# AdamCodd/local-hyperDB

Measured on AMD Instinct MI355X. Metric: queries/sec, N=10M d=384 fp16 top-100 (single-query stream; p50 latency alongside), higher is better.
Workload: dtype f16; 1 GPU; N=10000000 d=384 fp16 Q=1 cosine_similarity top-100, row-sharded x1; rows_per_gpu=10000000, accumulate=f32, exchange=none

## Files before the change

local-hyperdb_amd/csrc/hdb_api.hip:

```cpp
#include "hdb_common.h"
#include "hdb_quant.h"
#include "hdb_ws.h"
#include "hdb_plan.h"
#include "../../include/hyperdb_hip.h"
#include <string>
#include <cmath>
#include <cstring>
#include <cstdio>
#include <algorithm>
#include <vector>
#include <chrono>
#include <atomic>

static thread_local std::string g_err;
static int fail(int code, const std::string& msg) { g_err = msg; return code; }
#define HIP_TRY(expr)                                                                              \
    do {                                                                                           \
        hipError_t e_ = (expr);                                                                    \
        if (e_ != hipSuccess)                                                                      \
            return fail(HDB_ERR_HIP, std::string(#expr) + ": " + hipGetErrorString(e_));           \
    } while (0)
#define LAUNCH_TRY(expr)                                                                           \
    do {                                                                                           \
        int e_ = (expr);                                                                           \
// ... 31 lines not shown
    uint32_t fused_epoch = 0;
    char* bctl = nullptr;
    char* rec = nullptr;
    size_t rec_bytes = 0;
    int qmode = HDB_QUANT_NONE;
    int8_t* qcodes = nullptr;
    float* qaux = nullptr;
    int64_t q_rows = 0;
    int32_t qP = 0;
    int* qstat = nullptr;
    uint8_t* pnib = nullptr;
    uint32_t* pbit = nullptr;
    float* prec = nullptr;
    int32_t pU = 0;
    bool plane_declined = false;
    bool qauto = false;
    bool qauto_declined = false;
    char* ws = nullptr;
    size_t ws_bytes = 0;
    hdb_options opt;
    int flags_host = -1;
    TopkStats st;
    int64_t st_host_direct = 0;
    const uint32_t* qb_cnt = nullptr;
    int qb_cnt_n = 0;
    int64_t ht_pre_ns = 0, ht_launch_ns = 0, ht_wait_ns = 0, ht_calls = 0;
    std::chrono::steady_clock::time_point ht_l0, ht_l1;
    int64_t ht_attr_ns = 0;
    int64_t profile = 0;
    std::vector<hipEvent_t> ev_pool;
    size_t ev_used = 0;
};

static int ensure_ws(hdb_index* ix, size_t bytes) {
    if (bytes <= ix->ws_bytes) return HDB_OK;
    if (ix->ws) { HIP_TRY(hipDeviceSynchronize()); HIP_TRY(hipFree(ix->ws)); ix->ws = nullptr; ix->ws_bytes = 0; }
    bytes = align_up(bytes + (bytes >> 2), 1 << 20);
    HIP_TRY(hipMalloc((void**)&ix->ws, bytes));
    ix->ws_bytes = bytes;
    return HDB_OK;
}
template <typename WS, typename... Ext>
static int ws_lay(hdb_index* ix, WS& w, Ext... ext) {
    const int rc = ensure_ws(ix, ws_bytes_for<WS>(ext...));
    if (rc) return rc;
    Bump b(ix->ws, ix->ws_bytes);
    w.lay(b, ext...);
    if (b.off > b.cap) return fail(HDB_ERR_NOMEM, "workspace: a layout ran past the size it reported");
    return HDB_OK;
}

extern "C" int hdb_version(void) { return 107; }
extern "C" const char* hdb_last_error(void) { return g_err.c_str(); }

static int build_caches(hdb_index* ix, hipStream_t st) {
    if (ix->n > ix->cache_rows) {
        if (ix->inv_norm) { HIP_TRY(hipDeviceSynchronize()); HIP_TRY(hipFree(ix->inv_norm)); HIP_TRY(hipFree(ix->sqnorm)); }
        const int64_t rows = ix->n + ix->n / 4 + 64;
        HIP_TRY(hipMalloc((void**)&ix->inv_norm, rows * sizeof(float)));
        HIP_TRY(hipMalloc((void**)&ix->sqnorm, rows * sizeof(float)));
        ix->cache_rows = rows;
    }
    HIP_TRY(hipMemsetAsync(ix->nan_flag, 0, sizeof(int), st));
    if (ix->n > 0) LAUNCH_TRY(hdb_launch_rownorm(ix->V, ix->n, ix->d, ix->dtype, ix->inv_norm, ix->sqnorm, ix->nan_flag, st));
    ix->flags_host = -1;
    ix->bits_valid = false; ix->bits_done = 0;
    ix->pscale_valid = false; ix->pscale_done = 0;
    ix->build_stream = st;
    return HDB_OK;
}

static double quant_gamma(int d) {
    const double u = std::ldexp(1.0, -24), m = (double)(d + 8) * u;
    return m / (1.0 - m) * (1.0 + std::ldexp(1.0, -20));
}
// ... 344 lines not shown
    else if (!strcmp(name, "host_poll")) ix->opt.host_poll = value;
    else if (!strcmp(name, "dyn_tiles")) ix->opt.dyn_tiles = value;
    else if (!strcmp(name, "dyn_min_mb")) ix->opt.dyn_min_mb = std::max<int64_t>(0, value);
    else if (!strcmp(name, "dyn_heavy")) ix->opt.dyn_heavy = value;
    else if (!strcmp(name, "fused_timeout_us")) ix->opt.fused_timeout_us = std::max<int64_t>(1, value);
    else if (!strcmp(name, "bits_fused")) ix->opt.bits_fused = value;
    else if (!strcmp(name, "bits_local")) ix->opt.bits_local = value;
    else if (!strcmp(name, "fused_max_q")) ix->opt.fused_max_q = value;
    else if (!strcmp(name, "f32_min_q")) ix->opt.f32_min_q = value;
    else if (!strcmp(name, "f32_split")) ix->opt.f32_split = value;
    else if (!strcmp(name, "f32_split_min_q")) ix->opt.f32_split_min_q = value;
    else if (!strcmp(name, "bf16_ks_min_q")) ix->opt.bf16_ks_min_q = value;
    else if (!strcmp(name, "f8_ks_min_q")) ix->opt.f8_ks_min_q = value < 0 ? -1 : value;
    else if (!strcmp(name, "f8_lds_min_q")) ix->opt.f8_lds_min_q = value < 0 ? -1 : value;
    else if (!strcmp(name, "bf16_quant")) ix->opt.bf16_quant = value ? 1 : 0;
    else if (!strcmp(name, "f8_lds_waves")) { if (value == 0 || value == 4 || value == 8) ix->opt.f8_lds_waves = value; }
    else if (!strcmp(name, "bits_max_q")) ix->opt.bits_max_q = value;
    else if (!strcmp(name, "use_quant")) ix->opt.use_quant = value;
    else if (!strcmp(name, "quant_min_n")) ix->opt.quant_min_n = value;
    else if (!strcmp(name, "auto_quant")) ix->opt.auto_quant = value;
    else if (!strcmp(name, "quant_batch_min_n")) ix->opt.quant_batch_min_n = value;
    else if (!strcmp(name, "quant_batch_kernel")) ix->opt.quant_batch_kernel = value ? 1 : 0;
    else if (!strcmp(name, "quant_max_k")) ix->opt.quant_max_k = std::max<int64_t>(1, std::min<int64_t>(value, 128));
    else if (!strcmp(name, "use_plane")) ix->opt.use_plane = value;
    else if (!strcmp(name, "plane_min_n")) ix->opt.plane_min_n = value;
    else if (!strcmp(name, "plane_cap_rows")) ix->opt.plane_cap_rows = std::max<int64_t>(0, value);
    else if (!strcmp(name, "plane_wg_per_cu")) ix->opt.plane_wg_per_cu = std::max<int64_t>(0, std::min<int64_t>(value, 8));
    else if (!strcmp(name, "use_subset")) ix->opt.use_subset = value;
    else if (!strcmp(name, "subset_min_n")) ix->opt.subset_min_n = value < 0 ? -1 : value;
    else if (!strcmp(name, "subset_ratio")) ix->opt.subset_ratio = value < 0 ? -1 : std::max<int64_t>(1, value);
    else if (!strcmp(name, "profile")) { ix->profile = value; ix->ev_used = 0; }
    else if (!strcmp(name, "host_timing_reset")) { ix->ht_pre_ns = ix->ht_launch_ns = ix->ht_wait_ns = ix->ht_calls = ix->ht_attr_ns = 0; }
    else return fail(HDB_ERR_ARG, std::string("hdb_set_option: unknown option ") + name);
    return HDB_OK;
}

extern "C" int hdb_get_stat(hdb_index* ix, const char* name, int64_t* value) {
    if (!ix || !name || !value) return fail(HDB_ERR_ARG, "hdb_get_stat: null argument");
    if (!strcmp(name, "sample_rows")) *value = ix->st.sample_rows;
    else if (!strcmp(name, "sample_m")) *value = ix->st.sample_m;
    else if (!strcmp(name, "path")) *value = ix->st.path;
    else if (!strcmp(name, "chunks")) *value = ix->st.chunks;
    else if (!strcmp(name, "mfma")) *value = ix->st.mfma;
    else if (!strcmp(name, "f32_split")) *value = ix->st.f32s;
    else if (!strcmp(name, "f8_lds")) *value = ix->st.f8_lds;
    else if (!strcmp(name, "f8_lds_min_q")) *value = f8_lds_first_q(ix->opt, ix->dtype, ix->d);
    else if (!strcmp(name, "host_direct")) *value = ix->st_host_direct;
    else if (!strcmp(name, "fused")) *value = ix->st.fused;
    else if (!strcmp(name, "local")) *value = ix->st.local;
    else if (!strcmp(name, "cand_cap")) *value = HDB_CAND_CAP;
    else if (!strcmp(name, "quant")) *value = ix->st.quant;
    else if (!strcmp(name, "quant_auto")) *value = (ix->qmode == HDB_QUANT_I8 && ix->qauto) ? 1 : 0;
    else if (!strcmp(name, "quant_bytes")) *value = ix->qmode == HDB_QUANT_I8 ? ix->n * (int64_t)(ix->qP + 12) : 0;
    else if (!strcmp(name, "plane")) *value = ix->st.plane;
    else if (!strcmp(name, "plane_blocks")) *value = ix->st.plane_blocks;
    else if (!strcmp(name, "subset")) *value = ix->st.subset;
    else if (!strcmp(name, "subset_rows")) *value = ix->subset_m;
    else if (!strcmp(name, "plane_bytes")) *value = (ix->qmode == HDB_QUANT_I8 && ix->pnib) ? ix->n * (int64_t)plane_row_bytes(ix->qP) : 0;
    else if (!strcmp(name, "plane_survivors") || !strcmp(name, "plane_overflows")) {
        int h[HDB_QSTAT_WORDS] = {0, 0, 0, 0};
        if (ix->qstat) {
            HIP_TRY(hipSetDevice(ix->device));
            HIP_TRY(hipDeviceSynchronize());
            HIP_TRY(hipMemcpy(h, ix->qstat, sizeof(h), hipMemcpyDeviceToHost));
        }
        *value = name[6] == 's' ? (ix->st.plane ? (int64_t)(uint32_t)h[1] : 0) : (int64_t)(uint32_t)h[2];
    }
    else if (!strcmp(name, "quant_cands")) {
        int h = 0;
        if (ix->st.quant && ix->qstat) {
            HIP_TRY(hipSetDevice(ix->device));
            HIP_TRY(hipDeviceSynchronize());
            HIP_TRY(hipMemcpy(&h, ix->qstat, sizeof(int), hipMemcpyDeviceToHost));
        }
        *value = h;
    }
// ... 194 lines not shown
    }
    if (p.plane_wanted && !ix->pnib) {
        const int rc = plane_rows(ix, 0, ix->n, st);
        if (rc) return rc;
        *declined = ix->pnib == nullptr;
    }
    return HDB_OK;
}

static int quant_topk(hdb_index* ix, const TopkArgs& c, const TopkPlan& p) {
    const void* dev_Q = c.Q; const int32_t nq = c.nq, k = c.k; const int metric = c.metric; hipStream_t st = c.st;
    int64_t* dev_idx = c.idx; float* dev_score = c.score; int32_t* dev_status = c.status;
    const uint32_t kk = p.kk; const bool mflavour = p.mflavour, use_pl = p.plane_wanted;
    const int64_t n = ix->n;
    const uint32_t m = 16;
    const QuantSample sp = p.qs;
    QuantWs w;
    int rc = quant_ws_lay(ix, w, nq, quant_hi_cap(ix, nq), mflavour);
    if (rc) return rc;
    uint32_t* qstat = reinterpret_cast<uint32_t*>(ix->qstat);
    uint32_t* pl_cnt = use_pl ? qstat + 1 : nullptr;
    const size_t crow = (size_t)nq * HDB_CAND_CAP;
    const int nsub = p.nsub;
    rc = quant_query_prep(ix, (const float*)dev_Q, nq, w, mflavour, ix->qstat, nsub ? w.cnt : nullptr, pl_cnt, st);
    if (rc) return rc;
    QuantArgs a; quant_base_args(ix, a, w.qcodes, w.qaux, w.qinv, metric, nq);
    a.ntiles = sp.s_tiles; a.tile_stride = sp.s_stride; a.scores = w.sbuf; a.ld = sp.ld_s;
    a.wmax = w.wmax; a.nsub = nsub; a.thr_out = w.thr;
    a.pl_hi = use_pl ? reinterpret_cast<float*>(w.pl_list) : nullptr;
    if (use_pl && (!a.pl_hi || sp.s_rows > (int64_t)quant_hi_cap(ix, nq))) return fail(HDB_ERR_ARG, "quant_topk: no list for the sampled rows");
    LAUNCH_TRY(hdb_launch_quant_scan(&a, 0, (int)ix->opt.max_blocks, st));
    if (!nsub) LAUNCH_TRY(hdb_launch_sample_thr(w.sbuf, sp.s_rows, sp.ld_s, nq, m, w.thr, w.cnt, nullptr, st));
    a.ntiles = (n + 15) / 16; a.tile_stride = 1; a.scores = nullptr; a.ld = 0;
    a.thr = w.thr; a.cnt = w.cnt; a.cand = w.cand; a.cap = HDB_CAND_CAP;
    const bool has_bias = ix->bias != nullptr || ix->mask != nullptr;
    if (mflavour) {
        a.V = (const char*)ix->V; a.row_bytes = ix->d * 2; a.G = w.G;
        a.ginv = metric == HDB_COSINE ? w.ginv : nullptr; a.gbias = has_bias ? w.gbias : nullptr;
    }
    prof_begin(ix, st);
    if (use_pl) {
        a.pl_nib = ix->pnib; a.pl_bit = ix->pbit; a.pl_rec = ix->prec; a.pl_units = ix->pU;
        a.pl_cnt = pl_cnt; a.pl_cap = p.pl_cap;
        a.pl_s_tiles = (uint32_t)sp.s_tiles; a.pl_s_stride = (uint32_t)sp.s_stride;
        LAUNCH_TRY(hdb_launch_quant_plane_scan(&a, 0, p.pl_blocks, st));
    } else {
        LAUNCH_TRY(hdb_launch_quant_scan(&a, 1, (int)ix->opt.max_blocks, st));
    }
    prof_end(ix, st);
    if (mflavour) {
        ScanArgs s; memset(&s, 0, sizeof(s));
        s.V = w.G; s.n = (int64_t)crow; s.d = ix->d; s.Q = dev_Q; s.metric = metric; s.inv_norm = w.ginv; s.qinv = w.qinv;
        s.bias = has_bias ? w.gbias : nullptr; s.mask = nullptr; s.nq = nq;
        s.tile_stride = 1; s.ntiles = (int64_t)crow / hdb_mfma_tile_rows(ix->dtype, ix->d); s.cap = HDB_CAND_CAP;
        s.scores = w.gsc; s.ld = (int64_t)crow;
        LAUNCH_TRY(hdb_launch_mfma_scan(&s, ix->dtype, 0, nq, w.q16, w.ginv, w.qsq, w.qscl, (int)ix->opt.max_blocks, (int)ix->opt.mfma_variant, st, nullptr));
    } else {
        LAUNCH_TRY(hdb_launch_quant_rescore(ix->V, ix->d, ix->dtype, (const float*)dev_Q, nq, metric, ix->inv_norm, w.qinv, ix->bias, ix->mask,
                                            w.cand, w.cnt, HDB_CAND_CAP, st));
    }
    LAUNCH_TRY(hdb_launch_quant_finalize(w.cand, w.cnt, HDB_CAND_CAP, nq, (uint32_t)k, kk, ix->row_base, dev_idx, dev_score, dev_status, w.qnan,
                                         w.qaux, w.thr, ix->qstat, mflavour ? w.cand : nullptr, w.gsc, (int64_t)crow, st));
    return HDB_OK;
}

extern "C" int hdb_debug_quant_bounds(hdb_index* ix, const float* dev_q, int metric, float* dev_hi, float* dev_hi5, void* stream) {
    if (!ix || !dev_q || !dev_hi || !dev_hi5) return fail(HDB_ERR_ARG, "hdb_debug_quant_bounds: null argument");
    if (metric != HDB_DOT && metric != HDB_COSINE) return fail(HDB_ERR_ARG, "hdb_debug_quant_bounds: dot or cosine");
    if (ix->qmode != HDB_QUANT_I8 || !ix->pnib || ix->n < 1) return fail(HDB_ERR_UNSUPPORTED, "hdb_debug_quant_bounds: the index has no 5-bit plane");
    HIP_TRY(hipSetDevice(ix->device));
    hipStream_t st = (hipStream_t)stream;
    QuantWs w;
    int rc = quant_ws_lay(ix, w, 1, quant_hi_cap(ix, 1), true);
    if (rc) return rc;
    rc = quant_query_prep(ix, dev_q, 1, w, ix->qauto, nullptr, nullptr, nullptr, st);
    if (rc) return rc;
    QuantArgs a; quant_base_args(ix, a, w.qcodes, w.qaux, w.qinv, metric, 1);
    a.ntiles = (ix->n + 15) / 16; a.tile_stride = 1;
    a.pl_nib = ix->pnib; a.pl_bit = ix->pbit; a.pl_rec = ix->prec; a.pl_units = ix->pU;
    a.dbg = dev_hi;
    LAUNCH_TRY(hdb_launch_quant_scan_one(&a, 2, (int)ix->opt.max_blocks, st));
    a.dbg = dev_hi5;
    LAUNCH_TRY(hdb_launch_quant_plane_scan(&a, 1, hdb_quant_plane_dbg_blocks(a.ntiles, (int)ix->opt.max_blocks), st));
    return HDB_OK;
}
// ... 291 lines not shown
static int topk_impl(hdb_index* ix, const void* dev_Q, int32_t nq, int32_t k, int metric, int64_t* dev_idx,
                     float* dev_score, int32_t* dev_status, void* stream, bool exact) {
    if (!ix || !dev_idx || !dev_score) return fail(HDB_ERR_ARG, "hdb_topk: null argument");
    if (nq < 0 || k < 0) return fail(HDB_ERR_ARG, "hdb_topk: nq and k must be >= 0");
    if (nq == 0 || k == 0) return HDB_OK;
    if (!dev_Q) return fail(HDB_ERR_ARG, "hdb_topk: query pointer is null");
    if (metric == HDB_EUCLIDEAN_DIST || !metric_ok(metric)) return fail(HDB_ERR_UNSUPPORTED, "hdb_topk: metric not built");
    if (metric == HDB_PEARSON && ix->d < 1) return fail(HDB_ERR_ARG, "hdb_topk: pearson needs d >= 1");
    HIP_TRY(hipSetDevice(ix->device));
    const TopkArgs c{dev_Q, nq, k, metric, dev_idx, dev_score, dev_status, (hipStream_t)stream};
    const TopkCall call{nq, k, metric, dev_status != nullptr, exact};
    int frc = HDB_OK;
    auto finite = [&] { bool f = false; if (frc == HDB_OK) frc = matrix_is_finite(ix, &f); return f; };
    TopkPlan p = plan_topk(topk_facts(ix), ix->opt, call, finite);
    if (frc != HDB_OK) return frc;
    if (p.shadow()) {
        bool declined = false;
        const int rc = shadow_prepare(ix, p, nq, c.st, &declined);
        if (rc) return rc;
        if (declined) p = plan_topk(topk_facts(ix), ix->opt, call, finite);
        if (frc != HDB_OK) return frc;
    }
    ix->st = p.stats;
    ix->qb_cnt = nullptr; ix->qb_cnt_n = 0;
    switch (p.path) {
    case HDB_PATH_EMPTY: return run_empty(c);
    case HDB_PATH_QUANT: return quant_topk(ix, c, p);
    case HDB_PATH_QUANT_BATCH: return quant_batch_topk(ix, c, p);
    case HDB_PATH_FUSED: return run_fused(ix, c, p);
    case HDB_PATH_BITS1: return run_bits1(ix, c, p);
    case HDB_PATH_BATCH1: return run_batch1(ix, c, p);
    case HDB_PATH_FULL_SORT: return run_full_sort(ix, c, p);
    case HDB_PATH_PIPELINE: return run_pipeline(ix, c, p);
    }
    return fail(HDB_ERR_ARG, "hdb_topk: no path");
}

extern "C" int hdb_topk(hdb_index* ix, const void* dev_Q, int32_t nq, int32_t k, int metric, int64_t* dev_idx,
                        float* dev_score, int32_t* dev_status, void* stream) {
    return topk_impl(ix, dev_Q, nq, k, metric, dev_idx, dev_score, dev_status, stream, false);
}

static void merge_host_records(const char* const* recs, int32_t parts, int32_t nq, int32_t k, void* out_record) {
    int64_t* oi = reinterpret_cast<int64_t*>(out_record);
    float* os = reinterpret_cast<float*>(static_cast<char*>(out_record) + (int64_t)nq * k * 8);
    int32_t* ost = reinterpret_cast<int32_t*>(static_cast<char*>(out_record) + (int64_t)nq * k * 12);
    std::vector<int32_t> pos((size_t)parts);
// ... 364 lines not shown
```

local-hyperdb_amd/csrc/hdb_plan.h:

```cpp
#pragma once
#include "hdb_ws.h"
#include <algorithm>

struct hdb_options {
    int64_t max_blocks = 0;
    int64_t force_exact = 0;
    int64_t sample_target = 0;
    int64_t mfma_min_q = 1;
    int64_t use_mfma = 1;
    int64_t exact_bytes = (int64_t)1 << 30;
    int64_t bits_fused = 1;
    int64_t bits_local = 1;
    int64_t fused_max_q = -1;
    int64_t f32_min_q = -1;
    int64_t f32_split = 1;
    int64_t f32_split_min_q = -1;
    int64_t bf16_ks_min_q = -1;
    int64_t f8_ks_min_q = 0;
    int64_t f8_lds_min_q = 0;
    int64_t bf16_quant = 0;
    int64_t f8_lds_waves = 0;
    int64_t bits_max_q = -1;
    int64_t host_direct = 1;
    int64_t dyn_tiles = 1;
    int64_t dyn_min_mb = 16;
    int64_t dyn_heavy = 0;
    int64_t host_poll = 1;
    int64_t use_fused = 1;
    int64_t use_local = 1;
    int64_t local_m = 0;
    int64_t local_max_tiles = 4;
    int64_t local_small = 0;
    int64_t local_max_q = 1;
    int64_t use_l1_tile = 1;
    int64_t l1_packed = 1;
    int64_t use_batch1 = 1;
    int64_t fused_timeout_us = 2000;
    int64_t finalize_threads = 1024;
    int64_t mfma_variant = 16;
    int64_t use_quant = 1;
    int64_t quant_min_n = -1;
    int64_t quant_max_k = 128;
    int64_t auto_quant = 1;
    int64_t quant_batch_min_n = -1;
    int64_t quant_batch_kernel = 1;
    int64_t use_plane = 1;
    int64_t plane_min_n = -1;
    int64_t plane_cap_rows = 0;
    int64_t plane_wg_per_cu = 0;
    int64_t use_subset = 1;
    int64_t subset_min_n = -1;
    int64_t subset_ratio = -1;
};

struct TopkFacts {
    int64_t n; int32_t d; int dtype;
    int qmode;
    bool qauto;
    bool qauto_declined;
    bool plane_present, plane_declined;
    bool has_mask, has_bias;
    int cus;
    int64_t subset_m;
};
struct TopkCall { int32_t nq, k; int metric; bool has_status, exact; };

enum TopkPath {
    HDB_PATH_EMPTY,
// ... 261 lines not shown
```

local-hyperdb_amd/csrc/hdb_quant.h:

```cpp
#pragma once
#include <stdint.h>

#define HDB_QROW_S 0
#define HDB_QROW_E 1
#define HDB_QROW_T 2
#define HDB_QQ_S 0
#define HDB_QQ_N 1
#define HDB_QQ_D 2
#define HDB_QQ_SQ 3
#define HDB_QQ_BAD 4
#define HDB_QQ_CN 5
#define HDB_QQ_CS 6
#define HDB_QQ_WORDS 8

struct QuantArgs {
    const int8_t* codes;
    int64_t n;
    int32_t d;
    int32_t P;
    const float* aux;
    const float* sqnorm;
    const float* inv_norm;
    const int8_t* qcodes;
    const float* qaux;
    const float* qinv;
    const float* bias;
    const uint8_t* mask;
    int32_t metric;
    int32_t nq;
    float gamma;
    int64_t ntiles;
    int64_t tile_stride;
    float* scores; int64_t ld;
    const float* thr; uint32_t* cnt; unsigned long long* cand; uint32_t cap;
    uint32_t* wmax; int32_t nsub; float* thr_out;
    const char* V; int32_t row_bytes; char* G; float* ginv; float* gbias;
    const uint8_t* pl_nib; const uint32_t* pl_bit; const float* pl_rec; int32_t pl_units;
    uint32_t* pl_cnt; uint32_t pl_cap;
    float* pl_hi; uint32_t pl_s_tiles; uint32_t pl_s_stride;
    float* dbg;
};
#define HDB_QUANT_NSUB_MAX 4096
```

local-hyperdb_amd/csrc/hdb_quant.hip:

```cpp
#include "hdb_common.h"
#include "hdb_quant.h"
#include "hdb_finalize.h"
#include "../../include/hyperdb_hip.h"

__device__ __forceinline__ float hq_up(double x) {
    x = x * (1.0 + 0x1p-40);
    float f = (float)x;
    if ((double)f < x) f = nextafterf(f, INFINITY);
    return f;
}

__device__ __forceinline__ float hq_f(__half v) { return __half2float(v); }
__device__ __forceinline__ float hq_f(hdb_bf16 v) { return hdb_bf16_to_f(v); }
__device__ __forceinline__ float hq_f(float v) { return v; }

template <typename T> struct HqElem;
template <> struct HqElem<__half> { static constexpr int EPC = 8; };
template <> struct HqElem<hdb_bf16> { static constexpr int EPC = 8; };
template <> struct HqElem<float> { static constexpr int EPC = 4; };

__device__ __forceinline__ void hq_unpack(const uint4& raw, float (&x)[8], __half*) {
    const __half2* h = reinterpret_cast<const __half2*>(&raw);
#pragma unroll
    for (int i = 0; i < 4; ++i) { float2 f = __half22float2(h[i]); x[2 * i] = f.x; x[2 * i + 1] = f.y; }
// ... 107 lines not shown
        qcodes[(int64_t)q * P + e] = (int8_t)c;
        cs += c; c2 += c * c;
    }
#pragma unroll
    for (int o = 32; o > 0; o >>= 1) {
        nn += __shfl_xor(nn, o, 64); dd += __shfl_xor(dd, o, 64);
        cs += __shfl_xor(cs, o, 64); c2 += __shfl_xor(c2, o, 64);
    }
    if (lane == 0) {
        float* o = qaux + (int64_t)q * HDB_QQ_WORDS;
        const float sq = (float)nn;
        const bool big = !(sq - sq == 0.f);
        o[HDB_QQ_S] = s;
        o[HDB_QQ_N] = bad ? 0.f : hq_up(sqrt(nn));
        o[HDB_QQ_D] = bad ? 0.f : hq_up(sqrt(dd));
        o[HDB_QQ_SQ] = sq;
        o[HDB_QQ_BAD] = (bad || big) ? 1.f : 0.f;
        o[HDB_QQ_CN] = hq_up(sqrt((double)c2));
        o[HDB_QQ_CS] = (float)cs;
        o[7] = 0.f;
    }
}

__global__ __launch_bounds__(64) void hdb_quant_qprep_m_kernel(const float* Q, int nq, int d, int P, float* qinv, float* qsq, int* qnan,
                                                               _Float16* q16, float* qscl, int8_t* qcodes, float* qaux, int* stat,
                                                               uint32_t* cnt_init, uint32_t* pl_cnt) {
    const int q = blockIdx.x, lane = threadIdx.x;
    if (q >= nq) return;
    if (q == 0 && lane == 0 && stat) stat[0] = 0;
    if (q == 0 && lane == 0 && pl_cnt) pl_cnt[0] = 0u;
    if (lane == 0 && cnt_init) cnt_init[q * HDB_CNT_STRIDE] = 0u;
    const float* qr = Q + (int64_t)q * d;
    float s = 0.f, amax = 0.f;
    bool bad = false;
    for (int e = lane; e < d; e += 64) {
        const float x = qr[e];
        s = fma(x, x, s);
        amax = fmaxf(amax, fabsf(x));
        if (!(x - x == 0.f)) bad = true;
    }
#pragma unroll
    for (int o = 32; o > 0; o >>= 1) amax = fmaxf(amax, __shfl_xor(amax, o, 64));
    const float scale = hdb_q16_scale(amax);
    const float inv_scale = 1.f / scale;
    float amax2 = 0.f;
    for (int e = lane; e < d; e += 64) {
        const _Float16 h = (_Float16)(qr[e] * scale);
        q16[(int64_t)q * d + e] = h;
        const float xr = (float)h * inv_scale;
        if (!(xr - xr == 0.f)) bad = true;
        amax2 = fmaxf(amax2, fabsf(xr));
    }
#pragma unroll
    for (int o = 32; o > 0; o >>= 1) { s += __shfl_xor(s, o, 64); amax2 = fmaxf(amax2, __shfl_xor(amax2, o, 64)); }
    bad = __ballot(bad) != 0ull;
    const float sq_ = bad ? 0.f : amax2 / 127.f;
    double nn = 0.0, dd = 0.0;
    int cs = 0, c2 = 0;
    for (int e = lane; e < P; e += 64) {
        int c = 0;
        if (e < d && !bad) {
            const double x = (double)((float)(_Float16)(qr[e] * scale) * inv_scale);
            c = hq_code(x, sq_);
            const double del = x - (double)sq_ * (double)c;
            nn += x * x;
            dd += del * del;
        }
        qcodes[(int64_t)q * P + e] = (int8_t)c;
        cs += c; c2 += c * c;
    }
#pragma unroll
    for (int o = 32; o > 0; o >>= 1) {
        nn += __shfl_xor(nn, o, 64); dd += __shfl_xor(dd, o, 64);
        cs += __shfl_xor(cs, o, 64); c2 += __shfl_xor(c2, o, 64);
    }
    if (lane == 0) {
        const float ss = s;
        qsq[q] = ss;
        qinv[q] = (s == 0.f) ? 1.0f : (float)(1.f / sqrt(s));
        qnan[q] = (ss != ss) ? 1 : (ss - ss != 0.f) ? 2 : 0;
        qscl[q] = inv_scale;
        float* o = qaux + (int64_t)q * HDB_QQ_WORDS;
        const float sq = (float)nn;
        const bool big = !(sq - sq == 0.f);
        o[HDB_QQ_S] = sq_;
        o[HDB_QQ_N] = bad ? 0.f : hq_up(sqrt(nn));
        o[HDB_QQ_D] = bad ? 0.f : hq_up(sqrt(dd));
        o[HDB_QQ_SQ] = sq;
        o[HDB_QQ_BAD] = (bad || big) ? 1.f : 0.f;
        o[HDB_QQ_CN] = hq_up(sqrt((double)c2));
        o[HDB_QQ_CS] = (float)cs;
        o[7] = 0.f;
    }
}

#define HQ_STAGE_CAP 128
struct HqStage {
    unsigned long long buf[4][HQ_STAGE_CAP];
    unsigned int cnt[4];
    unsigned int base;
};

__device__ __forceinline__ int hq_dpp_i(int x, int ctrl_id) {
    switch (ctrl_id) {
    case 0: return __builtin_amdgcn_update_dpp(0, x, HDB_DPP_MIRROR, 0xF, 0xF, false);
    case 1: return __builtin_amdgcn_update_dpp(0, x, HDB_DPP_HALF_MIRROR, 0xF, 0xF, false);
    case 2: return __builtin_amdgcn_update_dpp(0, x, HDB_DPP_XOR2, 0xF, 0xF, false);
    default: return __builtin_amdgcn_update_dpp(0, x, HDB_DPP_XOR1, 0xF, 0xF, false);
    }
}
__device__ __forceinline__ int hq_rows4_sum(int a0, int a1, int a2, int a3, int l16) {
    const bool b3 = (l16 & 8) != 0, b2 = (l16 & 4) != 0;
    const int v01 = (b3 ? a1 : a0) + hq_dpp_i(b3 ? a0 : a1, 0);
    const int v23 = (b3 ? a3 : a2) + hq_dpp_i(b3 ? a2 : a3, 0);
    int w = (b2 ? v23 : v01) + hq_dpp_i(b2 ? v01 : v23, 1);
    w += hq_dpp_i(w, 2);
// ... 190 lines not shown
        }
    }
}
template <int NQ>
__device__ __forceinline__ void hq_stage_flush(HqStage& stage) {
    __syncthreads();
    const QuantArgs& a = hq_args_in_memory();
    for (int q = 0; q < NQ; ++q) {
        const unsigned int have = min(stage.cnt[q], (unsigned int)HQ_STAGE_CAP);
        if (have == 0u) continue;
        if (threadIdx.x == 0) stage.base = atomicAdd(&a.cnt[q * HDB_CNT_STRIDE], have);
        __syncthreads();
        const unsigned int base = stage.base;
        for (unsigned int e = threadIdx.x; e < have; e += blockDim.x)
            if (base + e < a.cap) a.cand[(int64_t)q * a.cap + base + e] = stage.buf[q][e];
        if (a.G)
            for (unsigned int e = threadIdx.x >> 6; e < have; e += blockDim.x >> 6)
                if (base + e < a.cap)
                    hq_copy_row(a, (int64_t)q * a.cap + base + e, 0xFFFFFFFFu - (uint32_t)(stage.buf[q][e] & 0xFFFFFFFFull), threadIdx.x & 63, 64);
        __syncthreads();
    }
}

template <int MODE, int NQ, int NJ>
__global__ __launch_bounds__(256) void hdb_quant_scan_kernel(QuantArgs a) {
    static_assert(sizeof(QuantArgs) % 8 == 0, "the argument block is read back from the kernarg segment as laid out here");
    extern __shared__ __attribute__((aligned(16))) char smem[];
    int4* qs = reinterpret_cast<int4*>(smem);
    __shared__ HqStage stage;
    const int nch = a.P >> 4;
    if (MODE == 1 && threadIdx.x < 4) stage.cnt[threadIdx.x] = 0u;
    for (int i = threadIdx.x; i < NQ * nch; i += 256) qs[i] = reinterpret_cast<const int4*>(a.qcodes)[i];
    HqQuery<NQ> qc;
    hq_query_load<NQ>(a, qc);
    float q_thr[NQ];
#pragma unroll
    for (int q = 0; q < NQ; ++q) q_thr[q] = (MODE == 1 && a.nsub == 0) ? a.thr[q] : 0.f;
    __syncthreads();
    if (MODE == 1 && a.nsub > 0) hq_fold_thr<NQ>(a, q_thr);

    const int lane = threadIdx.x & 63, wave = threadIdx.x >> 6;
    const int g = lane >> 4, l16 = lane & 15;
    uint32_t wbest[NQ];
#pragma unroll
    for (int q = 0; q < NQ; ++q) wbest[q] = 0u;

    const int64_t ntiles = a.ntiles;
    for (int64_t t = (int64_t)blockIdx.x * 4 + wave; t < ntiles; t += (int64_t)gridDim.x * 4) {
        const int64_t r0 = hdb_tile_index(t, a.tile_stride) * 16 + 4 * g;
        const int64_t rr[4] = {r0, r0 + 1, r0 + 2, r0 + 3};
        const int u_own = hdb_owned_row(l16);
        const int64_t row = r0 + u_own;
        const int64_t out_i = t * 16 + 4 * g + u_own;
        const bool live = hq_rows4_bounds<NQ, NJ, (NJ > 0 ? NJ : 2)>(a, qs, qc, rr, l16, row, [&](int q, float lo, float hi, bool masked) {
            if (MODE == 2) {
                a.dbg[row] = hi;
            } else if (MODE == 0) {
                if (a.nsub > 0) wbest[q] = max(wbest[q], hdb_f2key(lo));
                else a.scores[(int64_t)q * a.ld + out_i] = lo;
                if (NQ == 1 && a.pl_hi) a.pl_hi[out_i] = hi;
            } else if (!masked && !qc.bad[q] && hi >= q_thr[q]) {
// ... 382 lines not shown
}

extern "C" int hdb_launch_quant_gather(const int8_t* codes, const float* aux, const int64_t* rows, int64_t m, int P, int8_t* codes_out,
                                       float* aux_out, void* stream) {
    if (m <= 0) return 0;
    hipLaunchKernelGGL(hdb_quant_gather_kernel, dim3(hdb_grid_for(m, 4, 8192)), dim3(256), 0, (hipStream_t)stream, codes, aux, rows, m, P,
                       codes_out, aux_out);
    return (int)hipGetLastError();
}

extern "C" int hdb_launch_quant_qprep(const float* Q, int nq, int d, int P, int8_t* qcodes, float* qaux, int* stat, uint32_t* pl_cnt,
                                      void* stream) {
    hipLaunchKernelGGL(hdb_quant_qprep_kernel, dim3(nq), dim3(64), 0, (hipStream_t)stream, Q, nq, d, P, qcodes, qaux, stat, pl_cnt);
    return (int)hipGetLastError();
}

extern "C" int hdb_launch_quant_qprep_m(const float* Q, int nq, int d, int P, float* qinv, float* qsq, int* qnan, void* q16, float* qscl,
                                        int8_t* qcodes, float* qaux, int* stat, uint32_t* cnt_init, uint32_t* pl_cnt, void* stream) {
    hipLaunchKernelGGL(hdb_quant_qprep_m_kernel, dim3(nq), dim3(64), 0, (hipStream_t)stream, Q, nq, d, P, qinv, qsq, qnan, (_Float16*)q16,
                       qscl, qcodes, qaux, stat, cnt_init, pl_cnt);
    return (int)hipGetLastError();
}

template <int MODE, int NQ>
static void hq_launch_scan_nq(const QuantArgs& a, int blocks, size_t lds, hipStream_t st) {
    const int nch = a.P >> 4;
    const int nj = (nch + 15) >> 4;
    if (nj == 1) hipLaunchKernelGGL((hdb_quant_scan_kernel<MODE, NQ, 1>), dim3(blocks), dim3(256), lds, st, a);
    else if (nj == 2) hipLaunchKernelGGL((hdb_quant_scan_kernel<MODE, NQ, 2>), dim3(blocks), dim3(256), lds, st, a);
    else if (nj == 3) hipLaunchKernelGGL((hdb_quant_scan_kernel<MODE, NQ, 3>), dim3(blocks), dim3(256), lds, st, a);
    else hipLaunchKernelGGL((hdb_quant_scan_kernel<MODE, NQ, 0>), dim3(blocks), dim3(256), lds, st, a);
}
template <int MODE>
static void hq_launch_scan_mode(const QuantArgs& a, int blocks, size_t lds, hipStream_t st) {
    switch (a.nq) {
    case 1: hq_launch_scan_nq<MODE, 1>(a, blocks, lds, st); break;
    case 2: hq_launch_scan_nq<MODE, 2>(a, blocks, lds, st); break;
    case 3: hq_launch_scan_nq<MODE, 3>(a, blocks, lds, st); break;
    default: hq_launch_scan_nq<MODE, 4>(a, blocks, lds, st); break;
    }
}
static bool hq_copy_args_ok(const QuantArgs& a) {
    return !a.G || (a.V && a.row_bytes > 0 && a.row_bytes % 16 == 0 && (reinterpret_cast<uintptr_t>(a.V) & 15) == 0 && (reinterpret_cast<uintptr_t>(a.G) & 15) == 0);
}
extern "C" int hdb_launch_quant_scan(const QuantArgs* args, int mode, int max_blocks, void* stream) {
    const QuantArgs& a = *args;
    if (a.nq < 1 || a.nq > 4 || (a.P & 15) != 0) return (int)hipErrorInvalidValue;
    const size_t lds = (size_t)a.nq * a.P;
    const int blocks = hdb_quant_scan_blocks(a.ntiles, max_blocks);
    if (a.nsub != 0 && (a.nsub > HDB_QUANT_NSUB_MAX || !a.wmax || (mode == 0 ? a.nsub != 4 * blocks : !a.thr_out))) return (int)hipErrorInvalidValue;
    if (mode == 0) hq_launch_scan_mode<0>(a, blocks, lds, (hipStream_t)stream);
    else {
        if (!hq_copy_args_ok(a)) return (int)hipErrorInvalidValue;
        hq_launch_scan_mode<1>(a, blocks, lds, (hipStream_t)stream);
    }
    return (int)hipGetLastError();
}

extern "C" int hdb_launch_quant_plane_rows(const int8_t* codes, const float* aux, int64_t row0, int64_t m, int d, int P, uint8_t* nib,
                                           uint32_t* bitw, float* rec, void* stream) {
    if (m <= 0) return 0;
    const int U = hdb_quant_plane_units(P);
    if (U > 16 || (P & 15) != 0) return (int)hipErrorInvalidValue;
    hipLaunchKernelGGL(hdb_quant_plane_rows_kernel, dim3(hdb_grid_for(m, 16, 8192)), dim3(256), 0, (hipStream_t)stream, codes, aux, row0, m, d,
                       P, U, nib, bitw, rec);
    return (int)hipGetLastError();
}
extern "C" int hdb_launch_quant_plane_scan(const QuantArgs* args, int dbg, int blocks, void* stream) {
    const QuantArgs& a = *args;
    const int U = a.pl_units;
    if (blocks < 1 || blocks > (1 << 22)) return (int)hipErrorInvalidValue;
    if (a.nq != 1 || U < 1 || U > 16 || U != hdb_quant_plane_units(a.P) || (a.metric != HDB_DOT && a.metric != HDB_COSINE)) return (int)hipErrorInvalidValue;
    if (!dbg && a.nsub != 0 && (a.nsub > HDB_QUANT_NSUB_MAX || !a.wmax || !a.thr_out)) return (int)hipErrorInvalidValue;
    if (!dbg && (!a.cnt || !a.cand || !a.pl_cnt || !hq_copy_args_ok(a))) return (int)hipErrorInvalidValue;
// ... 67 lines not shown
```

profiles/summarize.py:

```python
#!/usr/bin/env python3
import csv
import glob
import json
import os
import sys


def find(d, suffix):
    hits = glob.glob(os.path.join(d, "**", "*" + suffix), recursive=True)
    if not hits:
        raise SystemExit(f"no *{suffix} under {d}")
    return hits[0]


def stats(src, dst):
    rows = list(csv.DictReader(open(find(src, "_kernel_stats.csv"))))
    with open(dst, "w", newline="") as f:
        w = csv.writer(f)
        w.writerow(["Name", "Calls", "TotalDurationNs", "AverageNs", "Percentage", "MinNs", "MaxNs", "StdDev"])
        for r in rows:
            w.writerow([r["Name"][:110], r["Calls"], r["TotalDurationNs"], r["AverageNs"], r["Percentage"],
                        r["MinNs"], r["MaxNs"], r["StdDev"]])
    print("wrote", dst, len(rows), "kernels")

# ... 7 lines not shown
    for r in rows:
        name = r["Kernel_Name"]
        if "hdb_" not in name:
            continue
        by.setdefault(name, []).append(int(r["End_Timestamp"]) - int(r["Start_Timestamp"]))
    names = sorted(by)
    dem = subprocess.run(["c++filt"], input="\n".join(names), capture_output=True, text=True).stdout.split("\n")
    with open(dst, "w", newline="") as f:
        w = csv.writer(f)
        w.writerow(["Name", "Cluster", "Calls", "AverageNs", "MinNs", "MaxNs"])
        for name, dn in zip(names, dem):
            d = sorted(by[name])
            cl, cur = [], [d[0]]
            for x in d[1:]:
                if x > cur[-1] * ratio:
                    cl.append(cur); cur = [x]
                else:
                    cur.append(x)
            cl.append(cur)
            short = (dn or name).split("(")[0][:110]
            for i, c in enumerate(cl):
                w.writerow([short, i, len(c), round(sum(c) / len(c), 1), c[0], c[-1]])
    print("wrote", dst)


def pmc(fetch_dir, write_dir, needle, dst):
    def avg(d, counter):
        vals = [float(r["Counter_Value"])
                for path in glob.glob(os.path.join(d, "**", "*_counter_collection.csv"), recursive=True)
                for r in csv.DictReader(open(path))
                if needle in r["Kernel_Name"] and r["Counter_Name"] == counter]
        return (sum(vals) / len(vals), len(vals)) if vals else (0.0, 0)
    f, nf = avg(fetch_dir, "FETCH_SIZE")
    w, nw = avg(write_dir, "WRITE_SIZE")
    out = {
        "kernel": needle, "dispatches_fetch": nf, "dispatches_write": nw,
        "FETCH_SIZE_KiB_raw": f, "WRITE_SIZE_KiB_raw": w,
        "read_bytes_corrected": f * 1024 * 2, "write_bytes": w * 1024,
        "hbm_bytes_per_launch": f * 1024 * 2 + w * 1024,
        "correction": "FETCH_SIZE x1024 x2 (gfx950 counts 128-B requests as 64 B on wide streaming reads), WRITE_SIZE x1024",
    }
    json.dump(out, open(dst, "w"), indent=1)
    print(json.dumps(out))


def mfma(needle, flop, dst, dirs):
# ... 23 lines not shown
        out["clock_formula"] = "GRBM_GUI_ACTIVE / 8 / duration_ns"
        if flop:
            mfma_cycles = flop / 16384.0 * 16.0
            out["mfma_busy_frac_from_flop"] = mfma_cycles / (1024.0 * cyc)
            out["tflops_profiled"] = flop / dur_ns / 1e3
    if "SQ_VALU_MFMA_BUSY_CYCLES" in avg and avg.get("SQ_BUSY_CU_CYCLES"):
        out["mfma_busy_frac"] = avg["SQ_VALU_MFMA_BUSY_CYCLES"] / (avg["SQ_BUSY_CU_CYCLES"] * 4.0)
        out["mfma_busy_formula"] = "SQ_VALU_MFMA_BUSY_CYCLES / (SQ_BUSY_CU_CYCLES * 4)"
    if "SQ_VALU_MFMA_BUSY_CYCLES" in avg and gui:
        out["mfma_busy_frac_vs_gui"] = avg["SQ_VALU_MFMA_BUSY_CYCLES"] / (1024.0 * gui / 8.0)
    if avg.get("SQ_WAVE_CYCLES"):
        for k in ("SQ_WAIT_ANY", "SQ_WAIT_INST_ANY", "SQ_WAIT_INST_LDS", "SQ_ACTIVE_INST_ANY"):
            if k in avg:
                out[k + "_share_of_wave_cycles"] = avg[k] / avg["SQ_WAVE_CYCLES"]
    json.dump(out, open(dst, "w"), indent=1)
    print(json.dumps(out, indent=1))


if __name__ == "__main__":
    if sys.argv[1] == "stats":
        stats(sys.argv[2], sys.argv[3])
    elif sys.argv[1] == "legs":
        legs(sys.argv[2], sys.argv[3])
    elif sys.argv[1] == "mfma":
        mfma(sys.argv[2], float(sys.argv[3]), sys.argv[4], sys.argv[5:])
    else:
        pmc(sys.argv[2], sys.argv[3], sys.argv[4], sys.argv[5])
```

Before: 2031 queries/s.

## Fold per-query quant prep into the sample scan kernel to drop a launch

Moves the query quantization prep (norm, fp16 scaling, int8 codes, aux record) into the sample-pass scan kernel. Each block recomputes the prep into LDS, and only block 0 writes the global outputs. This removes one kernel launch and its dependency gap from the per-query chain, which matters at Q=1. In exchange every block repeats a small per-query computation and the scan kernel gains extra template variants and register pressure. It also adds a launch counter stat and a trace-summarising script.

```diff
diff --git a/local-hyperdb_amd/csrc/hdb_api.hip b/local-hyperdb_amd/csrc/hdb_api.hip
--- a/local-hyperdb_amd/csrc/hdb_api.hip
+++ b/local-hyperdb_amd/csrc/hdb_api.hip
@@ -77,6 +77,7 @@
     int flags_host = -1;
     TopkStats st;
     int64_t st_host_direct = 0;
+    int64_t st_quant_launches = 0;
     const uint32_t* qb_cnt = nullptr;
     int qb_cnt_n = 0;
     int64_t ht_pre_ns = 0, ht_launch_ns = 0, ht_wait_ns = 0, ht_calls = 0;
@@ -105,7 +106,7 @@
     return HDB_OK;
 }
 
-extern "C" int hdb_version(void) { return 107; }
+extern "C" int hdb_version(void) { return 108; }
 extern "C" const char* hdb_last_error(void) { return g_err.c_str(); }
 
 static int build_caches(hdb_index* ix, hipStream_t st) {
@@ -496,6 +497,7 @@
     else if (!strcmp(name, "quant_batch_min_n")) ix->opt.quant_batch_min_n = value;
     else if (!strcmp(name, "quant_batch_kernel")) ix->opt.quant_batch_kernel = value ? 1 : 0;
     else if (!strcmp(name, "quant_max_k")) ix->opt.quant_max_k = std::max<int64_t>(1, std::min<int64_t>(value, 128));
+    else if (!strcmp(name, "quant_fold")) ix->opt.quant_fold = std::max<int64_t>(0, std::min<int64_t>(value, 3));
     else if (!strcmp(name, "use_plane")) ix->opt.use_plane = value;
     else if (!strcmp(name, "plane_min_n")) ix->opt.plane_min_n = value;
     else if (!strcmp(name, "plane_cap_rows")) ix->opt.plane_cap_rows = std::max<int64_t>(0, value);
@@ -526,6 +528,7 @@
     else if (!strcmp(name, "quant")) *value = ix->st.quant;
     else if (!strcmp(name, "quant_auto")) *value = (ix->qmode == HDB_QUANT_I8 && ix->qauto) ? 1 : 0;
     else if (!strcmp(name, "quant_bytes")) *value = ix->qmode == HDB_QUANT_I8 ? ix->n * (int64_t)(ix->qP + 12) : 0;
+    else if (!strcmp(name, "quant_launches")) *value = ix->st_quant_launches;
     else if (!strcmp(name, "plane")) *value = ix->st.plane;
     else if (!strcmp(name, "plane_blocks")) *value = ix->st.plane_blocks;
     else if (!strcmp(name, "subset")) *value = ix->st.subset;
@@ -766,15 +769,26 @@
     uint32_t* pl_cnt = use_pl ? qstat + 1 : nullptr;
     const size_t crow = (size_t)nq * HDB_CAND_CAP;
     const int nsub = p.nsub;
-    rc = quant_query_prep(ix, (const float*)dev_Q, nq, w, mflavour, ix->qstat, nsub ? w.cnt : nullptr, pl_cnt, st);
-    if (rc) return rc;
+    int64_t& launches = ix->st_quant_launches;
+    const bool fold_prep = mflavour && (ix->opt.quant_fold & 1);
+    if (!fold_prep) {
+        rc = quant_query_prep(ix, (const float*)dev_Q, nq, w, mflavour, ix->qstat, nsub ? w.cnt : nullptr, pl_cnt, st);
+        if (rc) return rc;
+        launches += mflavour ? 1 : 2;
+    }
     QuantArgs a; quant_base_args(ix, a, w.qcodes, w.qaux, w.qinv, metric, nq);
     a.ntiles = sp.s_tiles; a.tile_stride = sp.s_stride; a.scores = w.sbuf; a.ld = sp.ld_s;
     a.wmax = w.wmax; a.nsub = nsub; a.thr_out = w.thr;
     a.pl_hi = use_pl ? reinterpret_cast<float*>(w.pl_list) : nullptr;
     if (use_pl && (!a.pl_hi || sp.s_rows > (int64_t)quant_hi_cap(ix, nq))) return fail(HDB_ERR_ARG, "quant_topk: no list for the sampled rows");
+    if (fold_prep) {
+        a.pq_Q = (const float*)dev_Q; a.pq_qinv = w.qinv; a.pq_qsq = w.qsq; a.pq_qnan = w.qnan; a.pq_q16 = w.q16; a.pq_qscl = w.qscl;
+        a.pq_qcodes = w.qcodes; a.pq_qaux = w.qaux; a.pq_stat = ix->qstat; a.pq_cnt_init = nsub ? w.cnt : nullptr; a.pq_pl_cnt = pl_cnt;
+    }
     LAUNCH_TRY(hdb_launch_quant_scan(&a, 0, (int)ix->opt.max_blocks, st));
-    if (!nsub) LAUNCH_TRY(hdb_launch_sample_thr(w.sbuf, sp.s_rows, sp.ld_s, nq, m, w.thr, w.cnt, nullptr, st));
+    a.pq_Q = nullptr;
+    ++launches;
+    if (!nsub) { LAUNCH_TRY(hdb_launch_sample_thr(w.sbuf, sp.s_rows, sp.ld_s, nq, m, w.thr, w.cnt, nullptr, st)); ++launches; }
     a.ntiles = (n + 15) / 16; a.tile_stride = 1; a.scores = nullptr; a.ld = 0;
     a.thr = w.thr; a.cnt = w.cnt; a.cand = w.cand; a.cap = HDB_CAND_CAP;
     const bool has_bias = ix->bias != nullptr || ix->mask != nullptr;
@@ -791,6 +805,7 @@
     } else {
         LAUNCH_TRY(hdb_launch_quant_scan(&a, 1, (int)ix->opt.max_blocks, st));
     }
+    ++launches;
     prof_end(ix, st);
     if (mflavour) {
         ScanArgs s; memset(&s, 0, sizeof(s));
@@ -805,6 +820,7 @@
     }
     LAUNCH_TRY(hdb_launch_quant_finalize(w.cand, w.cnt, HDB_CAND_CAP, nq, (uint32_t)k, kk, ix->row_base, dev_idx, dev_score, dev_status, w.qnan,
                                          w.qaux, w.thr, ix->qstat, mflavour ? w.cand : nullptr, w.gsc, (int64_t)crow, st));
+    launches += 2;
     return HDB_OK;
 }
 
@@ -1142,7 +1158,7 @@
         if (frc != HDB_OK) return frc;
     }
     ix->st = p.stats;
-    ix->qb_cnt = nullptr; ix->qb_cnt_n = 0;
+    ix->qb_cnt = nullptr; ix->qb_cnt_n = 0; ix->st_quant_launches = 0;
     switch (p.path) {
     case HDB_PATH_EMPTY: return run_empty(c);
     case HDB_PATH_QUANT: return quant_topk(ix, c, p);
diff --git a/local-hyperdb_amd/csrc/hdb_plan.h b/local-hyperdb_amd/csrc/hdb_plan.h
--- a/local-hyperdb_amd/csrc/hdb_plan.h
+++ b/local-hyperdb_amd/csrc/hdb_plan.h
@@ -44,6 +44,7 @@
     int64_t auto_quant = 1;
     int64_t quant_batch_min_n = -1;
     int64_t quant_batch_kernel = 1;
+    int64_t quant_fold = 3;
     int64_t use_plane = 1;
     int64_t plane_min_n = -1;
     int64_t plane_cap_rows = 0;
diff --git a/local-hyperdb_amd/csrc/hdb_quant.h b/local-hyperdb_amd/csrc/hdb_quant.h
--- a/local-hyperdb_amd/csrc/hdb_quant.h
+++ b/local-hyperdb_amd/csrc/hdb_quant.h
@@ -39,5 +39,7 @@
     uint32_t* pl_cnt; uint32_t pl_cap;
     float* pl_hi; uint32_t pl_s_tiles; uint32_t pl_s_stride;
     float* dbg;
+    const float* pq_Q; float* pq_qinv; float* pq_qsq; int32_t* pq_qnan; void* pq_q16; float* pq_qscl; int8_t* pq_qcodes; float* pq_qaux;
+    int32_t* pq_stat; uint32_t* pq_cnt_init; uint32_t* pq_pl_cnt;
 };
 #define HDB_QUANT_NSUB_MAX 4096
diff --git a/local-hyperdb_amd/csrc/hdb_quant.hip b/local-hyperdb_amd/csrc/hdb_quant.hip
--- a/local-hyperdb_amd/csrc/hdb_quant.hip
+++ b/local-hyperdb_amd/csrc/hdb_quant.hip
@@ -153,34 +153,49 @@
     }
 }
 
-__global__ __launch_bounds__(64) void hdb_quant_qprep_m_kernel(const float* Q, int nq, int d, int P, float* qinv, float* qsq, int* qnan,
-                                                               _Float16* q16, float* qscl, int8_t* qcodes, float* qaux, int* stat,
-                                                               uint32_t* cnt_init, uint32_t* pl_cnt) {
-    const int q = blockIdx.x, lane = threadIdx.x;
-    if (q >= nq) return;
-    if (q == 0 && lane == 0 && stat) stat[0] = 0;
-    if (q == 0 && lane == 0 && pl_cnt) pl_cnt[0] = 0u;
-    if (lane == 0 && cnt_init) cnt_init[q * HDB_CNT_STRIDE] = 0u;
+template <bool LDS>
+__device__ __forceinline__ void hq_qprep_m(int q, int lane, bool glob, const float* Q, int d, int P, float* qinv, float* qsq, int* qnan,
+                                           _Float16* q16, float* qscl, int8_t* qcodes, float* qaux, int* stat, uint32_t* cnt_init,
+                                           uint32_t* pl_cnt, int8_t* l_codes, float* l_rec) {
+    if (glob && q == 0 && lane == 0 && stat) stat[0] = 0;
+    if (glob && q == 0 && lane == 0 && pl_cnt) pl_cnt[0] = 0u;
+    if (glob && lane == 0 && cnt_init) cnt_init[q * HDB_CNT_STRIDE] = 0u;
     const float* qr = Q + (int64_t)q * d;
+    constexpr int RQ = 8;
+    const bool held = d <= 64 * RQ;
+    float xq[RQ];
+#pragma unroll
+    for (int i = 0; i < RQ; ++i) { const int e = lane + 64 * i; xq[i] = (held && e < d) ? qr[e] : 0.f; }
     float s = 0.f, amax = 0.f;
     bool bad = false;
-    for (int e = lane; e < d; e += 64) {
-        const float x = qr[e];
+    auto pass1 = [&](float x) {
         s = fma(x, x, s);
         amax = fmaxf(amax, fabsf(x));
         if (!(x - x == 0.f)) bad = true;
+    };
+    if (held) {
+#pragma unroll
+        for (int i = 0; i < RQ; ++i) if (lane + 64 * i < d) pass1(xq[i]);
+    } else {
+        for (int e = lane; e < d; e += 64) pass1(qr[e]);
     }
 #pragma unroll
     for (int o = 32; o > 0; o >>= 1) amax = fmaxf(amax, __shfl_xor(amax, o, 64));
     const float scale = hdb_q16_scale(amax);
     const float inv_scale = 1.f / scale;
     float amax2 = 0.f;
-    for (int e = lane; e < d; e += 64) {
-        const _Float16 h = (_Float16)(qr[e] * scale);
-        q16[(int64_t)q * d + e] = h;
+    auto pass2 = [&](int e, float x) {
+        const _Float16 h = (_Float16)(x * scale);
+        if (glob) q16[(int64_t)q * d + e] = h;
         const float xr = (float)h * inv_scale;
         if (!(xr - xr == 0.f)) bad = true;
         amax2 = fmaxf(amax2, fabsf(xr));
+    };
+    if (held) {
+#pragma unroll
+        for (int i = 0; i < RQ; ++i) if (lane + 64 * i < d) pass2(lane + 64 * i, xq[i]);
+    } else {
+        for (int e = lane; e < d; e += 64) pass2(e, qr[e]);
     }
 #pragma unroll
     for (int o = 32; o > 0; o >>= 1) { s += __shfl_xor(s, o, 64); amax2 = fmaxf(amax2, __shfl_xor(amax2, o, 64)); }
@@ -188,17 +203,24 @@
     const float sq_ = bad ? 0.f : amax2 / 127.f;
     double nn = 0.0, dd = 0.0;
     int cs = 0, c2 = 0;
-    for (int e = lane; e < P; e += 64) {
+    auto pass3 = [&](int e, float xe) {
         int c = 0;
         if (e < d && !bad) {
-            const double x = (double)((float)(_Float16)(qr[e] * scale) * inv_scale);
+            const double x = (double)((float)(_Float16)(xe * scale) * inv_scale);
             c = hq_code(x, sq_);
             const double del = x - (double)sq_ * (double)c;
             nn += x * x;
             dd += del * del;
         }
-        qcodes[(int64_t)q * P + e] = (int8_t)c;
+        if (glob) qcodes[(int64_t)q * P + e] = (int8_t)c;
+        if (LDS) l_codes[e] = (int8_t)c;
         cs += c; c2 += c * c;
+    };
+    if (held) {
+#pragma unroll
+        for (int i = 0; i < RQ; ++i) if (lane + 64 * i < P) pass3(lane + 64 * i, xq[i]);
+    } else {
+        for (int e = lane; e < P; e += 64) pass3(e, e < d ? qr[e] : 0.f);
     }
 #pragma unroll
     for (int o = 32; o > 0; o >>= 1) {
@@ -207,13 +229,10 @@
     }
     if (lane == 0) {
         const float ss = s;
-        qsq[q] = ss;
-        qinv[q] = (s == 0.f) ? 1.0f : (float)(1.f / sqrt(s));
-        qnan[q] = (ss != ss) ? 1 : (ss - ss != 0.f) ? 2 : 0;
-        qscl[q] = inv_scale;
-        float* o = qaux + (int64_t)q * HDB_QQ_WORDS;
+        const float inv = (s == 0.f) ? 1.0f : (float)(1.f / sqrt(s));
         const float sq = (float)nn;
         const bool big = !(sq - sq == 0.f);
+        float o[HDB_QQ_WORDS];
         o[HDB_QQ_S] = sq_;
         o[HDB_QQ_N] = bad ? 0.f : hq_up(sqrt(nn));
         o[HDB_QQ_D] = bad ? 0.f : hq_up(sqrt(dd));
@@ -222,7 +241,27 @@
         o[HDB_QQ_CN] = hq_up(sqrt((double)c2));
         o[HDB_QQ_CS] = (float)cs;
         o[7] = 0.f;
-    }
+        if (glob) {
+            qsq[q] = ss;
+            qinv[q] = inv;
+            qnan[q] = (ss != ss) ? 1 : (ss - ss != 0.f) ? 2 : 0;
+            qscl[q] = inv_scale;
+#pragma unroll
+            for (int i = 0; i < HDB_QQ_WORDS; ++i) qaux[(int64_t)q * HDB_QQ_WORDS + i] = o[i];
+        }
+        if (LDS) {
+#pragma unroll
+            for (int i = 0; i < HDB_QQ_WORDS; ++i) l_rec[i] = o[i];
+            l_rec[HDB_QQ_WORDS] = inv;
+        }
+    }
+}
+__global__ __launch_bounds__(64) void hdb_quant_qprep_m_kernel(const float* Q, int nq, int d, int P, float* qinv, float* qsq, int* qnan,
+                                                               _Float16* q16, float* qscl, int8_t* qcodes, float* qaux, int* stat,
+                                                               uint32_t* cnt_init, uint32_t* pl_cnt) {
+    const int q = blockIdx.x, lane = threadIdx.x;
+    if (q >= nq) return;
+    hq_qprep_m<false>(q, lane, true, Q, d, P, qinv, qsq, qnan, q16, qscl, qcodes, qaux, stat, cnt_init, pl_cnt, nullptr, nullptr);
 }
 
 #define HQ_STAGE_CAP 128
@@ -459,21 +498,39 @@
     }
 }
 
-template <int MODE, int NQ, int NJ>
+template <int MODE, int NQ, int NJ, bool PREP = false>
 __global__ __launch_bounds__(256) void hdb_quant_scan_kernel(QuantArgs a) {
     static_assert(sizeof(QuantArgs) % 8 == 0, "the argument block is read back from the kernarg segment as laid out here");
+    static_assert(!PREP || MODE == 0, "the query prep folds into the sample pass only");
     extern __shared__ __attribute__((aligned(16))) char smem[];
     int4* qs = reinterpret_cast<int4*>(smem);
     __shared__ HqStage stage;
     const int nch = a.P >> 4;
     if (MODE == 1 && threadIdx.x < 4) stage.cnt[threadIdx.x] = 0u;
-    for (int i = threadIdx.x; i < NQ * nch; i += 256) qs[i] = reinterpret_cast<const int4*>(a.qcodes)[i];
     HqQuery<NQ> qc;
-    hq_query_load<NQ>(a, qc);
     float q_thr[NQ];
-#pragma unroll
-    for (int q = 0; q < NQ; ++q) q_thr[q] = (MODE == 1 && a.nsub == 0) ? a.thr[q] : 0.f;
-    __syncthreads();
+    if constexpr (PREP) {
+        __shared__ float s_qrec[NQ][HDB_QQ_WORDS + 1];
+        const int pw = threadIdx.x >> 6;
+        if (pw < NQ)
+            hq_qprep_m<true>(pw, threadIdx.x & 63, blockIdx.x == 0, a.pq_Q, a.d, a.P, a.pq_qinv, a.pq_qsq, a.pq_qnan, (_Float16*)a.pq_q16,
+                             a.pq_qscl, a.pq_qcodes, a.pq_qaux, a.pq_stat, a.pq_cnt_init, a.pq_pl_cnt,
+                             reinterpret_cast<int8_t*>(smem) + pw * a.P, s_qrec[pw]);
+        __syncthreads();
+#pragma unroll
+        for (int q = 0; q < NQ; ++q) {
+            qc.s[q] = s_qrec[q][HDB_QQ_S]; qc.n[q] = s_qrec[q][HDB_QQ_N]; qc.d[q] = s_qrec[q][HDB_QQ_D]; qc.sq[q] = s_qrec[q][HDB_QQ_SQ];
+            qc.bad[q] = s_qrec[q][HDB_QQ_BAD] != 0.f;
+            qc.inv[q] = a.metric == HDB_COSINE ? s_qrec[q][HDB_QQ_WORDS] : 1.f;
+            q_thr[q] = 0.f;
+        }
+    } else {
+        for (int i = threadIdx.x; i < NQ * nch; i += 256) qs[i] = reinterpret_cast<const int4*>(a.qcodes)[i];
+        hq_query_load<NQ>(a, qc);
+#pragma unroll
+        for (int q = 0; q < NQ; ++q) q_thr[q] = (MODE == 1 && a.nsub == 0) ? a.thr[q] : 0.f;
+        __syncthreads();
+    }
     if (MODE == 1 && a.nsub > 0) hq_fold_thr<NQ>(a, q_thr);
 
     const int lane = threadIdx.x & 63, wave = threadIdx.x >> 6;
@@ -902,22 +959,22 @@
     return (int)hipGetLastError();
 }
 
-template <int MODE, int NQ>
+template <int MODE, int NQ, bool PREP>
 static void hq_launch_scan_nq(const QuantArgs& a, int blocks, size_t lds, hipStream_t st) {
     const int nch = a.P >> 4;
     const int nj = (nch + 15) >> 4;
-    if (nj == 1) hipLaunchKernelGGL((hdb_quant_scan_kernel<MODE, NQ, 1>), dim3(blocks), dim3(256), lds, st, a);
-    else if (nj == 2) hipLaunchKernelGGL((hdb_quant_scan_kernel<MODE, NQ, 2>), dim3(blocks), dim3(256), lds, st, a);
-    else if (nj == 3) hipLaunchKernelGGL((hdb_quant_scan_kernel<MODE, NQ, 3>), dim3(blocks), dim3(256), lds, st, a);
-    else hipLaunchKernelGGL((hdb_quant_scan_kernel<MODE, NQ, 0>), dim3(blocks), dim3(256), lds, st, a);
-}
-template <int MODE>
+    if (nj == 1) hipLaunchKernelGGL((hdb_quant_scan_kernel<MODE, NQ, 1, PREP>), dim3(blocks), dim3(256), lds, st, a);
+    else if (nj == 2) hipLaunchKernelGGL((hdb_quant_scan_kernel<MODE, NQ, 2, PREP>), dim3(blocks), dim3(256), lds, st, a);
+    else if (nj == 3) hipLaunchKernelGGL((hdb_quant_scan_kernel<MODE, NQ, 3, PREP>), dim3(blocks), dim3(256), lds, st, a);
+    else hipLaunchKernelGGL((hdb_quant_scan_kernel<MODE, NQ, 0, PREP>), dim3(blocks), dim3(256), lds, st, a);
+}
+template <int MODE, bool PREP = false>
 static void hq_launch_scan_mode(const QuantArgs& a, int blocks, size_t lds, hipStream_t st) {
     switch (a.nq) {
-    case 1: hq_launch_scan_nq<MODE, 1>(a, blocks, lds, st); break;
-    case 2: hq_launch_scan_nq<MODE, 2>(a, blocks, lds, st); break;
-    case 3: hq_launch_scan_nq<MODE, 3>(a, blocks, lds, st); break;
-    default: hq_launch_scan_nq<MODE, 4>(a, blocks, lds, st); break;
+    case 1: hq_launch_scan_nq<MODE, 1, PREP>(a, blocks, lds, st); break;
+    case 2: hq_launch_scan_nq<MODE, 2, PREP>(a, blocks, lds, st); break;
+    case 3: hq_launch_scan_nq<MODE, 3, PREP>(a, blocks, lds, st); break;
+    default: hq_launch_scan_nq<MODE, 4, PREP>(a, blocks, lds, st); break;
     }
 }
 static bool hq_copy_args_ok(const QuantArgs& a) {
@@ -929,7 +986,10 @@
     const size_t lds = (size_t)a.nq * a.P;
     const int blocks = hdb_quant_scan_blocks(a.ntiles, max_blocks);
     if (a.nsub != 0 && (a.nsub > HDB_QUANT_NSUB_MAX || !a.wmax || (mode == 0 ? a.nsub != 4 * blocks : !a.thr_out))) return (int)hipErrorInvalidValue;
-    if (mode == 0) hq_launch_scan_mode<0>(a, blocks, lds, (hipStream_t)stream);
+    if (mode == 0 && a.pq_Q) {
+        if (blocks < 1 || !a.pq_qinv || !a.pq_qsq || !a.pq_qnan || !a.pq_q16 || !a.pq_qscl || !a.pq_qcodes || !a.pq_qaux) return (int)hipErrorInvalidValue;
+        hq_launch_scan_mode<0, true>(a, blocks, lds, (hipStream_t)stream);
+    } else if (mode == 0) hq_launch_scan_mode<0>(a, blocks, lds, (hipStream_t)stream);
     else {
         if (!hq_copy_args_ok(a)) return (int)hipErrorInvalidValue;
         hq_launch_scan_mode<1>(a, blocks, lds, (hipStream_t)stream);
diff --git a/profiles/summarize.py b/profiles/summarize.py
--- a/profiles/summarize.py
+++ b/profiles/summarize.py
@@ -53,6 +53,50 @@
             for i, c in enumerate(cl):
                 w.writerow([short, i, len(c), round(sum(c) / len(c), 1), c[0], c[-1]])
     print("wrote", dst)
+
+
+def calls(src, dst=None, skip=10):
+    rows = []
+    for path in glob.glob(os.path.join(src, "**", "*_kernel_trace.csv"), recursive=True):
+        rows += list(csv.DictReader(open(path)))
+    ks = sorted(((int(r["Start_Timestamp"]), int(r["End_Timestamp"]), r["Kernel_Name"].split("(")[0][:60]) for r in rows
+                 if "hdb_" in r["Kernel_Name"]), key=lambda t: t[0])
+    groups, cur = [], []
+    for k in ks:
+        prep = "qprep_m_kernel" in k[2]
+        sample = "hdb_quant_scan_kernel<0" in k[2] or "hdb_quant_scan_kernelILi0E" in k[2]
+        if prep or (sample and not (cur and len(cur) == 1 and "qprep_m_kernel" in cur[0][2])):
+            if cur:
+                groups.append(cur)
+            cur = []
+        if cur or prep or sample:
+            cur.append(k)
+    if cur:
+        groups.append(cur)
+    seqs = {}
+    for g in groups:
+        seqs.setdefault(tuple(k[2] for k in g), []).append(g)
+    if not seqs:
+        raise SystemExit("no shadow call in the trace")
+    names, gs = max(seqs.items(), key=lambda kv: len(kv[1]))
+    gs = gs[skip:]
+    med = lambda v: sorted(v)[len(v) // 2] / 1e3
+    out = [f"calls {len(gs)} (of {len(groups)} groups; first {skip} dropped), {len(names)} launches each"]
+    tot = 0.0
+    for i, n in enumerate(names):
+        d = [g[i][1] - g[i][0] for g in gs]
+        tot += med(d)
+        out.append(f"  launch {i} {n:<60s} median {med(d):8.2f}  min {min(d) / 1e3:8.2f}  max {max(d) / 1e3:8.2f}")
+        if i + 1 < len(names):
+            gap = [g[i + 1][0] - g[i][1] for g in gs]
+            tot += med(gap)
+            out.append(f"  gap {i}->{i + 1} median {med(gap):8.2f}  min {min(gap) / 1e3:8.2f}  max {max(gap) / 1e3:8.2f}")
+    span = [g[-1][1] - g[0][0] for g in gs]
+    out.append(f"  sum of the medians {tot:8.2f}   span of a call: median {med(span):8.2f}  min {min(span) / 1e3:8.2f}  max {max(span) / 1e3:8.2f}")
+    text = "\n".join(out)
+    print(text)
+    if dst:
+        open(dst, "w").write(text + "\n")
 
 
 def pmc(fetch_dir, write_dir, needle, dst):
@@ -122,6 +166,8 @@
         stats(sys.argv[2], sys.argv[3])
     elif sys.argv[1] == "legs":
         legs(sys.argv[2], sys.argv[3])
+    elif sys.argv[1] == "calls":
+        calls(sys.argv[2], sys.argv[3] if len(sys.argv) > 3 else None)
     elif sys.argv[1] == "mfma":
         mfma(sys.argv[2], float(sys.argv[3]), sys.argv[4], sys.argv[5:])
     else:
```

Result: no change. 2030 queries/s (median of 2 runs) (-0.1%).
